# starkware-libs/stark-perpetual

Measured on AMD Instinct MI355X. Metric: pedersen_hashes_per_sec, higher is better.
Workload: dtype u32x9; 1 GPU; 2^16-leaf Pedersen Merkle rebuild per GPU (BASELINE.json configs[1]), 63 rebuilds in lockstep; tree_height=16, leaves_per_gpu=65536, calls_per_region=28, streams=2, window_bits=26, combine=none

## Files before the change

stark-perpetual_amd/csrc/pedersen.hip:

```cpp
#include <algorithm>
#include <cstdlib>
#include <cstring>
#include <map>
#include <vector>

#include "context.hpp"
#include "pedersen.hpp"
#include "quad.hpp"
#include "ragged_plan.hpp"

#ifndef SP_ACC_WAVES
#define SP_ACC_WAVES 1
#endif

namespace sp {

struct raw_aff {
  u256 x, y;
};
__device__ __forceinline__ raw_aff ld_raw(const aff_packed* e) {
  const uint4* q = reinterpret_cast<const uint4*>(e);
  const uint4 a = q[0], b = q[1], c = q[2], d = q[3];
  raw_aff r;
  r.x.w[0] = a.x; r.x.w[1] = a.y; r.x.w[2] = a.z; r.x.w[3] = a.w;
  r.x.w[4] = b.x; r.x.w[5] = b.y; r.x.w[6] = b.z; r.x.w[7] = b.w;
  r.y.w[0] = c.x; r.y.w[1] = c.y; r.y.w[2] = c.z; r.y.w[3] = c.w;
  r.y.w[4] = d.x; r.y.w[5] = d.y; r.y.w[6] = d.z; r.y.w[7] = d.w;
  return r;
}
__device__ __forceinline__ aff unpack_raw(const raw_aff& t) {
  aff r;
  r.x = fe_unpack(t.x);
  r.y = fe_unpack(t.y);
  return r;
}

struct bits512 {
  uint32_t w[16];
};
// ... 120 lines not shown
    acc = xyzz_mmadd<SP_SCAN_BULK>(unpack_raw(e0), q1);
    first = 2;
  } else {
    acc = xyzz_from_aff(unpack_raw(e0));
  }
  for (int i = first; i + 1 < nwin; ++i) {
    const aff q = signed_aff(n1, neg1);
    n1 = n2;
    neg1 = neg2;
    if (i + 2 < nwin) {
      const window_ref r = next_window(i + 2);
      n2 = ld_raw(r.entry);
      neg2 = r.negative;
    }
    acc = xyzz_madd<SP_SCAN_BULK>(acc, q);
  }
  if (nwin > 1) {
    fe X3, ZZ3;
    xyzz_madd_x_only<SP_SCAN_BULK>(acc, signed_aff(n1, neg1), X3, ZZ3);
    store_limbs(sX, plane, e, X3);
    store_limbs(sZZ, plane, e, ZZ3);
  } else {
    store_limbs(sX, plane, e, acc.X);
    store_limbs(sZZ, plane, e, acc.ZZ);
  }
  if (st != SP_HASH_OK) {
    if (status) status[e] = st;
    if (flag) atomicOr(flag, (unsigned)st);
  } else if (status) {
    status[e] = SP_HASH_OK;
  }
}

__global__ void __launch_bounds__(256, SP_ACC_WAVES)
ped_accumulate_kernel(const uint64_t* __restrict__ x, const uint64_t* __restrict__ y, size_t xstride,
                      size_t ystride, size_t n, const aff_packed* __restrict__ ped, int w0, int log2e,
                      int nwin, int32_t* __restrict__ sX, int32_t* __restrict__ sZZ,
                      uint8_t* __restrict__ status, unsigned* __restrict__ flag,
                      const int2* __restrict__ src, size_t plane) {
  bulk_accumulate(x, y, xstride, ystride, n, ped, w0, log2e, nwin, sX, sZZ, status, flag, src, plane,
                  (size_t)blockIdx.x * blockDim.x + threadIdx.x);
}

__device__ __forceinline__ fe shfl_xor_fe(const fe& v, int mask) {
  fe r;
#pragma unroll
  for (int i = 0; i < NL; ++i) r.l[i] = __shfl_xor(v.l[i], mask, 64);
  return r;
}
__device__ __forceinline__ uint32_t field_from_memory(const uint64_t* felt, int bit, int width) {
  const uint32_t* w = reinterpret_cast<const uint32_t*>(felt);
  const int wi = bit >> 5, sh = bit & 31;
  uint64_t two = (uint64_t)w[wi];
  if (wi + 1 < 8) two |= (uint64_t)w[wi + 1] << 32;
  return (uint32_t)(two >> sh) & ((1u << width) - 1u);
}
__device__ __forceinline__ uint32_t window_from_memory(const uint64_t* fx, const uint64_t* fy, int start,
                                                       int width) {
  if (start + width <= 252) return field_from_memory(fx, start, width);
  if (start >= 252) return field_from_memory(fy, start - 252, width);
  const int lo_n = 252 - start;
  return field_from_memory(fx, start, lo_n) | (field_from_memory(fy, 0, width - lo_n) << lo_n);
}

template <int LOG_L>
__device__ __forceinline__ xyzz split_accumulate(const uint64_t* fx, const uint64_t* fy, int sub,
                                                 const aff_packed* __restrict__ ped, int w0, int log2e,
                                                 int nwin) {
  constexpr int L = 1 << LOG_L;
  const int cnt_lo = nwin / L, extra = nwin % L;
  const int cnt = cnt_lo + (sub < extra ? 1 : 0);
  const int g0 = sub * cnt_lo + (sub < extra ? sub : extra);
  auto entry = [&](int g) {
    return window_entry(ped, g, window_from_memory(fx, fy, window_start(g, w0, log2e), window_width(g, w0, log2e)),
// ... 65 lines not shown
  u256 xa_plain;
  if (FUSED) {
    fe zz = acc.ZZ;
    if constexpr (LOG_L < 2) {
      if (fe_is_zero(zz)) {
        zz = FE_ONE_M;
        st = SP_HASH_UNHASHABLE;
      }
    }
    const fe zinv = fe_inv_shared_quad<(LOG_L >= 2 ? 0 : 2 - LOG_L), true>(zz, (int)(threadIdx.x & 3));
    if constexpr (LOG_L >= 2) {
      if (limbs_is_zero(zinv)) st = SP_HASH_UNHASHABLE;
    }
    xa_plain = fe_pack(fe_canon(fe_mul(acc.X, zinv)));
  }
  if (!active || sub != 0) return;
  if (!u256_lt(ld_u256(fx), U256_P) || !u256_lt(ld_u256(fy), U256_P)) st = SP_HASH_OUT_OF_RANGE;
  if (FUSED) {
    st_u256(out + 4 * e * ostride, xa_plain);
  } else {
    store_limbs(sX, plane, e, acc.X);
    store_limbs(sZZ, plane, e, acc.ZZ);
  }
  if (status) status[e] = st;
  if (st != SP_HASH_OK && flag) atomicOr(flag, (unsigned)st);
}

template <int LOG_L>
__global__ void __launch_bounds__(256, SP_ACC_WAVES)
ped_accumulate_mixed_kernel(const uint64_t* __restrict__ x, const uint64_t* __restrict__ y, size_t xstride,
                            size_t ystride, size_t n_bulk, size_t rem, unsigned bulk_blocks,
                            const aff_packed* __restrict__ ped, int w0, int log2e, int nwin,
                            int32_t* __restrict__ sX, int32_t* __restrict__ sZZ, uint8_t* __restrict__ status,
                            unsigned* __restrict__ flag, const int2* __restrict__ src, size_t plane) {
  if (blockIdx.x < bulk_blocks) {
    bulk_accumulate(x, y, xstride, ystride, n_bulk, ped, w0, log2e, nwin, sX, sZZ, status, flag, src, plane,
                    (size_t)blockIdx.x * blockDim.x + threadIdx.x);
    return;
  }
  constexpr int L = 1 << LOG_L;
  const size_t gt = (size_t)(blockIdx.x - bulk_blocks) * blockDim.x + threadIdx.x;
  const size_t e_raw = gt >> LOG_L;
  const int sub = (int)(gt & (L - 1));
  const bool active = e_raw < rem;
  const size_t e = n_bulk + (active ? e_raw : rem - 1);
  const uint64_t *fx, *fy;
  operand_pointers(x, y, xstride, ystride, src, e, fx, fy);
  const xyzz acc = split_accumulate<LOG_L>(fx, fy, sub, ped, w0, log2e, nwin);
  if (!active || sub != 0) return;
  uint8_t st = SP_HASH_OK;
  if (!u256_lt(ld_u256(fx), U256_P) || !u256_lt(ld_u256(fy), U256_P)) st = SP_HASH_OUT_OF_RANGE;
  store_limbs(sX, plane, e, acc.X);
  store_limbs(sZZ, plane, e, acc.ZZ);
  if (status) status[e] = st;
  if (st != SP_HASH_OK && flag) atomicOr(flag, (unsigned)st);
}

template <int LOG_Q, bool SPARSE>
__device__ __forceinline__ u256 quad_hash(const uint64_t* fx, const uint64_t* fy, int mode, const aff_packed* __restrict__ cpts,
                                          int cx, int cy, const aff_packed* __restrict__ ped, int w0, int log2e,
                                          int nwin_plan, int g, bool* unhashable) {
  constexpr int QUADS = 1 << LOG_Q;
  const int q = g >> 2, k = g & 3;
  int nwin = nwin_plan, first_real = 0;
  if constexpr (SPARSE) {
    nwin = mode == 0 ? nwin_plan : 1 + nwin_plan - (mode == 1 ? cx : cy);
    first_real = mode == 1 ? cx - 1 : (mode == 2 ? -1 : 0);
  }
  auto entry = [&](int v) {
    if constexpr (SPARSE) {
      if (mode != 0 && v == 0) return unpack_raw(ld_raw(cpts + (mode - 1)));
    }
    const int w = first_real + v;
    const window_ref r =
// ... 230 lines not shown
        if (st != SP_HASH_OK && flag) atomicOr(flag, (unsigned)st);
      }
    }
    __syncthreads();
    h = slot[grp];
  }
}

__global__ void __launch_bounds__(256)
ped_fold_ragged_scatter_kernel(const uint64_t* __restrict__ work, const uint64_t* __restrict__ lone, bool sided,
                               const uint32_t* __restrict__ off, const uint32_t* __restrict__ perm,
                               const uint32_t* __restrict__ step_off, const uint8_t* __restrict__ step_status, size_t n,
                               unsigned* __restrict__ flag, uint8_t* __restrict__ status, uint64_t* __restrict__ out,
                               const uint64_t* __restrict__ expect, size_t estride, uint8_t* __restrict__ verdict) {
  const size_t k = (size_t)blockIdx.x * blockDim.x + threadIdx.x;
  if (k >= n) return;
  const uint32_t c = perm[k];
  const uint32_t o0 = off[c], steps = off[c + 1] - o0 - (sided ? 0 : 1);
  uint8_t st = SP_HASH_OK;
  u256 v;
  if (steps == 0) {
    v = ld_u256(lone + 4 * (size_t)(sided ? c : o0));
    if (!u256_lt(v, U256_P)) st = SP_HASH_OUT_OF_RANGE;
    if (st != SP_HASH_OK && flag) atomicOr(flag, (unsigned)st);
  } else {
    v = ld_u256(work + 4 * k);
    for (uint32_t s = 0; s < steps; ++s) st |= step_status[(size_t)step_off[s] + k];
  }
  fold_result<true>(c, v, st, out, status, expect, estride, verdict);
}

__global__ void __launch_bounds__(256)
ped_top_kernel(uint64_t* __restrict__ cur, size_t n_in, int n_levels, const aff_packed* __restrict__ ped, int w0, int log2e,
               int nwin_plan, unsigned* __restrict__ flag) {
  constexpr int LANES = 32, GROUPS = 256 / LANES;
  __shared__ uint64_t slot[2][GROUPS][4];
  const int g = (int)(threadIdx.x % LANES), grp = (int)(threadIdx.x / LANES);
  const size_t b = blockIdx.x;
  const int chunk = 1 << n_levels;
  uint64_t* out = cur + 4 * n_in;
  size_t n_out = n_in >> 1;
  int share = 4 - n_levels;
  for (int t = 0; t < n_levels; ++t, ++share) {
    const int cnt = chunk >> (t + 1);
    const int i = grp >> share;
    const bool writer = g == 0 && (grp & ((1 << share) - 1)) == 0;
    const uint64_t *fx, *fy;
    if (t == 0) {
      fx = cur + 4 * ((size_t)chunk * b + 2 * (size_t)i);
      fy = fx + 4;
    } else {
      fx = slot[(t - 1) & 1][2 * i];
      fy = slot[(t - 1) & 1][2 * i + 1];
    }
    bool unhashable;
    const u256 xa = quad_hash<3, false>(fx, fy, 0, nullptr, 0, 0, ped, w0, log2e, nwin_plan, g, &unhashable);
    uint8_t st = unhashable ? SP_HASH_UNHASHABLE : SP_HASH_OK;
    if (t == 0 && writer && (!u256_lt(ld_u256(fx), U256_P) || !u256_lt(ld_u256(fy), U256_P))) st = SP_HASH_OUT_OF_RANGE;
    if (writer) {
      uint32_t* sl = reinterpret_cast<uint32_t*>(slot[t & 1][i]);
#pragma unroll
      for (int w = 0; w < 8; ++w) sl[w] = xa.w[w];
      st_u256(out + 4 * ((size_t)cnt * b + (size_t)i), xa);
      if (st != SP_HASH_OK && flag) atomicOr(flag, (unsigned)st);
    }
    __syncthreads();
    out += 4 * n_out;
    n_out >>= 1;
  }
}

__global__ void __launch_bounds__(256)
ped_finish_kernel(const int32_t* __restrict__ sX, int32_t* __restrict__ sZZ, int32_t* __restrict__ sPre,
                  size_t n, size_t T, uint64_t* __restrict__ out, size_t ostride,
                  uint8_t* __restrict__ status, unsigned* __restrict__ flag) {
  const size_t t = (size_t)blockIdx.x * blockDim.x + threadIdx.x;
  if (t >= T) return;
  const size_t cnt = t < n ? (n - t + T - 1) / T : 0;
  fe run = FE_ONE_M;
  if (cnt > 0) {
    fe znext = load_limbs(sZZ, n, t);
#pragma unroll 1
    for (size_t j = 0; j < cnt; ++j) {
      const size_t e = t + j * T;
      const fe z = znext;
      if (j + 1 < cnt) znext = load_limbs(sZZ, n, e + T);
      store_limbs(sPre, n, e, run);
      run = fe_mul(run, z);
    }
  }
  if (fe_is_zero(run)) {
    run = FE_ONE_M;
#pragma unroll 1
    for (size_t e = t; e < n; e += T) {
      fe z = load_limbs(sZZ, n, e);
      if (fe_is_zero(z)) {
        z = FE_ONE_M;
        store_limbs(sZZ, n, e, z);
        if (status) status[e] = SP_HASH_UNHASHABLE;
        if (flag) atomicOr(flag, (unsigned)SP_HASH_UNHASHABLE);
      }
      store_limbs(sPre, n, e, run);
      run = fe_mul(run, z);
    }
  }
  size_t e = cnt > 0 ? t + (cnt - 1) * T : 0;
  fe zn = run, pn = run, xn = run;
  if (cnt > 0) {
    zn = load_limbs(sZZ, n, e);
    pn = load_limbs(sPre, n, e);
    xn = load_limbs(sX, n, e);
  }
  fe inv = fe_inv_shared_quad<2, true>(run, (int)(threadIdx.x & 3));
#pragma unroll 1
  for (size_t j = cnt; j-- > 0;) {
    const fe z = zn, pre = pn, xv = xn;
    const size_t cur = t + j * T;
    if (j > 0) {
      zn = load_limbs(sZZ, n, cur - T);
      pn = load_limbs(sPre, n, cur - T);
      xn = load_limbs(sX, n, cur - T);
    }
    const fe zinv = fe_mul(inv, pre);
    inv = fe_mul(inv, z);
    const fe xa = fe_mul(xv, zinv);
    st_u256(out + 4 * cur * ostride, fe_pack(fe_canon(xa)));
  }
}

template <bool Z_IN_LDS>
__global__ void __launch_bounds__(256)
ped_finish_lds_kernel(const int32_t* __restrict__ sX, int32_t* __restrict__ sZZ, size_t n, size_t T,
                      uint64_t* __restrict__ out, size_t ostride, uint8_t* __restrict__ status,
                      unsigned* __restrict__ flag, int kmax) {
  extern __shared__ int32_t fin_lds[];
  int32_t* lpre = fin_lds;
  int32_t* lz = fin_lds + (size_t)kmax * NL * 256;
  auto lds_put = [&](int32_t* base, size_t j, const fe& v) {
#pragma unroll
    for (int k = 0; k < NL; ++k) base[((j * NL + k) << 8) + threadIdx.x] = v.l[k];
  };
  auto lds_get = [&](const int32_t* base, size_t j) {
    fe v;
#pragma unroll
    for (int k = 0; k < NL; ++k) v.l[k] = base[((j * NL + k) << 8) + threadIdx.x];
    return v;
  };
  const size_t t = (size_t)blockIdx.x * blockDim.x + threadIdx.x;
  if (t >= T) return;
  const size_t cnt = t < n ? (n - t + T - 1) / T : 0;
  fe run = FE_ONE_M;
  if (cnt > 0) {
    fe znext = load_limbs(sZZ, n, t);
#pragma unroll 1
    for (size_t j = 0; j < cnt; ++j) {
      const fe z = znext;
      if (j + 1 < cnt) znext = load_limbs(sZZ, n, t + (j + 1) * T);
      lds_put(lpre, j, run);
      if (Z_IN_LDS) lds_put(lz, j, z);
      run = fe_mul(run, z);
    }
  }
  if (fe_is_zero(run)) {
    run = FE_ONE_M;
    size_t j = 0;
#pragma unroll 1
    for (size_t e = t; e < n; e += T, ++j) {
      fe z = load_limbs(sZZ, n, e);
      if (fe_is_zero(z)) {
        z = FE_ONE_M;
        store_limbs(sZZ, n, e, z);
        if (status) status[e] = SP_HASH_UNHASHABLE;
        if (flag) atomicOr(flag, (unsigned)SP_HASH_UNHASHABLE);
      }
      lds_put(lpre, j, run);
      if (Z_IN_LDS) lds_put(lz, j, z);
      run = fe_mul(run, z);
    }
  }
  size_t e = cnt > 0 ? t + (cnt - 1) * T : 0;
  fe zn = run, xn = run;
  if (cnt > 0) {
    if (!Z_IN_LDS) zn = load_limbs(sZZ, n, e);
    xn = load_limbs(sX, n, e);
  }
  fe inv = fe_inv_shared_quad<2, true>(run, (int)(threadIdx.x & 3));
#pragma unroll 1
  for (size_t j = cnt; j-- > 0;) {
    const fe z = Z_IN_LDS ? lds_get(lz, j) : zn, xv = xn;
    const fe pre = lds_get(lpre, j);
    const size_t cur = t + j * T;
    if (j > 0) {
      if (!Z_IN_LDS) zn = load_limbs(sZZ, n, cur - T);
      xn = load_limbs(sX, n, cur - T);
    }
    const fe zinv = fe_mul(inv, pre);
    inv = fe_mul(inv, z);
    const fe xa = fe_mul(xv, zinv);
    st_u256(out + 4 * cur * ostride, fe_pack(fe_canon(xa)));
  }
}

__global__ void __launch_bounds__(128)
ped_point_kernel(const uint64_t* __restrict__ x, const uint64_t* __restrict__ y, size_t n,
                 const aff_packed* __restrict__ ped, int w0, int log2e, int nwin,
                 uint64_t* __restrict__ ox, uint64_t* __restrict__ oy, uint8_t* __restrict__ status) {
  size_t e = (size_t)blockIdx.x * blockDim.x + threadIdx.x;
  if (e >= n) e = n - 1;
  u256 sx = ld_u256(x + 4 * e);
  u256 sy = ld_u256(y + 4 * e);
  if (!u256_lt(sx, U256_P) || !u256_lt(sy, U256_P)) {
    status[e] = SP_HASH_OUT_OF_RANGE;
    return;
  }
  bits512 str = concat_xy(sx, sy);
  xyzz acc = xyzz_from_aff(ld_aff(ped + pop_bits(str, w0)));
  for (int g = 1; g < nwin; ++g) {
    const window_ref r = window_entry(ped, g, pop_bits(str, log2e + 1), w0, log2e);
    acc = xyzz_madd(acc, signed_aff(ld_raw(r.entry), r.negative));
  }
  if (fe_is_zero(acc.ZZ)) {
    status[e] = SP_HASH_UNHASHABLE;
    return;
  }
  const fe izzz = fe_inv(acc.ZZZ);
  st_u256(ox + 4 * e, fe_pack(fe_from_mont(fe_mul(acc.X, fe_sqr(fe_mul(acc.ZZ, izzz))))));
  st_u256(oy + 4 * e, fe_pack(fe_from_mont(fe_mul(acc.Y, izzz))));
// ... 107 lines not shown

static size_t g_finish_lanes = getenv("STARKPERP_FINISH_LANES") ? (size_t)atoll(getenv("STARKPERP_FINISH_LANES")) : 65536;
static size_t parse_split_lanes() {
  const char* e = getenv("STARKPERP_SPLIT_LANES");
  long long v = e ? atoll(e) : 65536;
  if (v < 256) v = 256;
  if (v > (1ll << 24)) v = 1ll << 24;
  return ((size_t)v + 255) & ~(size_t)255;
}
static size_t g_split_lanes = parse_split_lanes();
static bool g_finish_lds = getenv("STARKPERP_NO_FINISH_LDS") == nullptr;
static int finish_lds_ready() {
  static std::map<int, int> done;
  int dev = -1;
  if (hipGetDevice(&dev) != hipSuccess) return SP_ERR_HIP;
  auto it = done.find(dev);
  if (it != done.end()) return it->second;
  const int want = 16 * NL * 256 * (int)sizeof(int32_t);
  hipError_t e = hipFuncSetAttribute(reinterpret_cast<const void*>(ped_finish_lds_kernel<true>),
                                     hipFuncAttributeMaxDynamicSharedMemorySize, want);
  if (e == hipSuccess)
    e = hipFuncSetAttribute(reinterpret_cast<const void*>(ped_finish_lds_kernel<false>),
                            hipFuncAttributeMaxDynamicSharedMemorySize, want);
  if (e != hipSuccess) (void)hipGetLastError();
  return done[dev] = (e == hipSuccess ? SP_OK : SP_ERR_HIP);
}
static size_t finish_threads(size_t n) {
  size_t K = (n + g_finish_lanes - 1) / g_finish_lanes;
  if (K < 1) K = 1;
  if (K > 32) K = 32;
  return ((n + K - 1) / K + 3) & ~(size_t)3;
}

void release_ragged_stage();
void release_pedersen_state() {
  for (auto& kv : g_stream_scratch) kv.second.release();
  g_stream_scratch.clear();
  release_ragged_stage();
  for (hipEvent_t e : g_prof.ev) (void)hipEventDestroy(e);
  g_prof.ev.clear();
  g_prof.units.clear();
  g_prof.used = 0;
  g_prof.enabled = false;
}

void constant_window_counts(const PedPlan& p, int& cx, int& cy) {
  cx = cy = 0;
  for (int g = 0; g < p.nwin; ++g) {
    if (p.start[g] + p.bits[g] <= 252) ++cx;
    if (p.start[g] >= 252) ++cy;
  }
}
static bool sparse_class(const PedPlan& plan, int log_q, int& cx, int& cy) {
  if (!g_sparse_enabled || (log_q != 1 && log_q != 2)) return false;
  constant_window_counts(plan, cx, cy);
  const int shortest = 1 + plan.nwin - (cx > cy ? cx : cy);
  return cx >= 1 && cy >= 1 && shortest >= (2 << log_q);
}
int enqueue_partial_points(const uint64_t* felts, int count, aff_packed* out, hipStream_t st, bool* usable) {
  Context& c = ctx();
  int cx, cy;
  constant_window_counts(c.plan, cx, cy);
  *usable = cx >= 1 && cy >= 1 && count > 0;
  if (!*usable) return SP_OK;
  hipLaunchKernelGGL(ped_partial_kernel, dim3((unsigned)((2 * count + 63) / 64)), dim3(64), 0, st, felts, count, c.ped,
                     (int)c.plan.bits[0], c.plan.log2e, c.plan.nwin, cx, cy, out);
  SP_HIP(hipGetLastError());
  return SP_OK;
}

static int enqueue_pedersen_impl(const uint64_t* x, size_t xs, const uint64_t* y, size_t ys, uint64_t* out,
                                 size_t os, uint8_t* status, unsigned* flag, size_t n, hipStream_t st,
                                 const Scratch& s, const int2* src, const aff_packed* cpts);
int enqueue_pedersen(const uint64_t* x, size_t xs, const uint64_t* y, size_t ys, uint64_t* out,
                     size_t os, uint8_t* status, unsigned* flag, size_t n, hipStream_t st,
                     const Scratch& s, const int2* src) {
  return enqueue_pedersen_impl(x, xs, y, ys, out, os, status, flag, n, st, s, src, nullptr);
}
int enqueue_pedersen_sparse(const uint64_t* x, const uint64_t* y, uint64_t* out, unsigned* flag, size_t n,
                            hipStream_t st, const Scratch& s, const int2* src, const aff_packed* cpts) {
  return enqueue_pedersen_impl(x, 1, y, 1, out, 1, nullptr, flag, n, st, s, src, cpts);
}
static bool g_path_fusion = getenv("STARKPERP_NO_PATH_FUSION") == nullptr;
static bool g_top_fusion = getenv("STARKPERP_NO_TOP_FUSION") == nullptr;
static bool g_chain_fusion = getenv("STARKPERP_NO_CHAIN_FUSION") == nullptr;
int enqueue_pedersen_chain(const uint64_t* first, const uint64_t* words, long long word_stride, size_t n, size_t steps,
                           bool h_right, uint64_t* out, unsigned* flag, hipStream_t st, bool* done) {
  *done = false;
  Context& c = ctx();
  const int w0 = c.plan.bits[0], log2e = c.plan.log2e, nwin = c.plan.nwin;
  if (!g_chain_fusion || n == 0 || steps < 2 || steps > 0x7fffffffull) return SP_OK;
  const QuadShape q = quad_shape(n, nwin);
  if (q.log_q == 0) return SP_OK;
  dispatch_quad(q.log_q, false, [&](auto Q, auto) {
    hipLaunchKernelGGL((ped_chain_kernel<decltype(Q)::value>), dim3(q.blocks), dim3(256), 0, st, first, words, word_stride,
                       n, (int)steps, h_right, c.ped, w0, log2e, nwin, flag, out, q.dup);
  });
  SP_HIP(hipGetLastError());
  *done = true;
  return SP_OK;
}
int enqueue_pedersen_top(uint64_t* cur, size_t n_in, unsigned remaining, unsigned* flag, hipStream_t st, int* levels_done) {
  *levels_done = 0;
  Context& c = ctx();
  const int nwin = c.plan.nwin;
  if (!g_top_fusion || !g_quad_enabled || nwin > 64 || nwin < 16 || remaining < 2 || n_in / 2 > g_quad_max || n_in < 4) return SP_OK;
  const int L = remaining < 4 ? (int)remaining : 4;
  const unsigned blocks = (unsigned)(n_in >> L);
  hipLaunchKernelGGL(ped_top_kernel, dim3(blocks), dim3(256), 0, st, cur, n_in, L, c.ped, (int)c.plan.bits[0], c.plan.log2e,
                     nwin, flag);
  SP_HIP(hipGetLastError());
  *levels_done = L;
  return SP_OK;
}
int enqueue_pedersen_path(uint64_t* felts, const uint64_t* emp, unsigned* flag, size_t n, hipStream_t st,
                          const int2* src_all, const PathLevels& pl, const aff_packed* cpts_tree, bool* done) {
  *done = false;
  Context& c = ctx();
  const int w0 = c.plan.bits[0], log2e = c.plan.log2e, nwin = c.plan.nwin;
  if (!g_path_fusion || n == 0 || pl.n_levels < 2) return SP_OK;
  const QuadShape q = quad_shape(n, nwin);
  if (q.log_q == 0) return SP_OK;
  int cx = 0, cy = 0;
  const bool sparse = cpts_tree != nullptr && sparse_class(c.plan, q.log_q, cx, cy);
  dispatch_quad(q.log_q, sparse, [&](auto Q, auto S) {
    hipLaunchKernelGGL((ped_path_kernel<decltype(Q)::value, decltype(S)::value>), dim3(q.blocks), dim3(256), 0, st, felts,
                       emp, n, c.ped, w0, log2e, nwin, flag, src_all, pl, q.dup, sparse ? cpts_tree : nullptr, cx, cy);
  });
  SP_HIP(hipGetLastError());
  *done = true;
  return SP_OK;
}

static int enqueue_pedersen_impl(const uint64_t* x, size_t xs, const uint64_t* y, size_t ys, uint64_t* out,
                                 size_t os, uint8_t* status, unsigned* flag, size_t n, hipStream_t st,
                                 const Scratch& s, const int2* src, const aff_packed* cpts) {
  if (n == 0) return SP_OK;
  Context& c = ctx();
  bool prof = false;
  const int w0 = c.plan.bits[0], log2e = c.plan.log2e, nwin = c.plan.nwin;
  int log_l = 0;
  bool fused = false;
  if (g_split_enabled) {
    if (n * 8 <= g_split_lanes) log_l = 3;
    else if (n * 4 <= g_split_lanes) log_l = 2;
    else if (n * 2 <= g_split_lanes) log_l = 1;
    while (log_l > 0 && nwin < (2 << log_l)) --log_l;
  }
  const QuadShape q = quad_shape(n, nwin);
  if (q.log_q != 0) {
    int cx = 0, cy = 0;
    const bool sparse = cpts != nullptr && src != nullptr && sparse_class(c.plan, q.log_q, cx, cy);
    dispatch_quad(q.log_q, sparse, [&](auto Q, auto S) {
      hipLaunchKernelGGL((ped_quad_kernel<decltype(Q)::value, decltype(S)::value>), dim3(q.blocks), dim3(256), 0, st, x, y,
                         xs, ys, n, c.ped, w0, log2e, nwin, status, flag, src, out, os, q.dup, cpts, cx, cy);
    });
    fused = true;
  } else if (log_l == 0 && !(g_split_enabled && g_fuse_enabled && n <= 65536)) {
    size_t n_bulk = n, rem = 0;
    int rem_l = 0;
    if (g_level_split && g_split_enabled && n > g_split_lanes && (n % g_split_lanes) != 0 &&
        (n % g_split_lanes) * 2 <= g_split_lanes) {
      rem = n % g_split_lanes;
      rem_l = rem * 8 <= g_split_lanes ? 3 : (rem * 4 <= g_split_lanes ? 2 : 1);
      while (rem_l > 0 && nwin < (2 << rem_l)) --rem_l;
      if (rem_l == 0) rem = 0;
      n_bulk = n - rem;
    }
    if (rem == 0) {
      prof = g_prof.enabled && g_prof.used + 2 <= g_prof.ev.size() && n > 65536;
      if (prof) (void)hipEventRecord(g_prof.ev[g_prof.used], st);
      hipLaunchKernelGGL(ped_accumulate_kernel, dim3((unsigned)((n_bulk + 255) / 256)), dim3(256), 0, st, x, y, xs, ys,
                         n_bulk, c.ped, w0, log2e, nwin, s.X, s.ZZ, status, flag, src, n);
    } else {
      const unsigned bulk_blocks = (unsigned)(n_bulk / 256);
      const unsigned rblocks = (unsigned)(((rem << rem_l) + 255) / 256);
#define SP_LAUNCH_MIXED(LOGL)                                                                                     \
  hipLaunchKernelGGL((ped_accumulate_mixed_kernel<LOGL>), dim3(bulk_blocks + rblocks), dim3(256), 0, st, x, y, xs, \
                     ys, n_bulk, rem, bulk_blocks, c.ped, w0, log2e, nwin, s.X, s.ZZ, status, flag, src, n)
      if (rem_l == 3) SP_LAUNCH_MIXED(3);
      else if (rem_l == 2) SP_LAUNCH_MIXED(2);
      else SP_LAUNCH_MIXED(1);
#undef SP_LAUNCH_MIXED
    }
    if (prof) {
      (void)hipEventRecord(g_prof.ev[g_prof.used + 1], st);
      g_prof.units.push_back(n);
      g_prof.used += 2;
    }
  } else {
    const unsigned blocks = (unsigned)(((n << log_l) + 255) / 256);
    fused = g_fuse_enabled && (n << log_l) <= 65536;
#define SP_LAUNCH_SPLIT(LOGL, FUSEDV)                                                                      \
  hipLaunchKernelGGL((ped_accumulate_split_kernel<LOGL, FUSEDV>), dim3(blocks), dim3(256), 0, st, x, y, xs, \
                     ys, n, c.ped, w0, log2e, nwin, s.X, s.ZZ, status, flag, src, out, os, n)
    if (log_l == 0) SP_LAUNCH_SPLIT(0, true);
    else if (log_l == 3) { if (fused) SP_LAUNCH_SPLIT(3, true); else SP_LAUNCH_SPLIT(3, false); }
    else if (log_l == 2) { if (fused) SP_LAUNCH_SPLIT(2, true); else SP_LAUNCH_SPLIT(2, false); }
    else { if (fused) SP_LAUNCH_SPLIT(1, true); else SP_LAUNCH_SPLIT(1, false); }
#undef SP_LAUNCH_SPLIT
  }
  if (!fused) {
    const size_t T = finish_threads(n);
    const unsigned tpb = T >= 256 ? 256 : 64;
    const unsigned blocksB = (unsigned)((T + tpb - 1) / tpb);
    const size_t kmax = (n + T - 1) / T;
    if (g_finish_lds && tpb == 256 && kmax >= 2 && kmax <= 16 && finish_lds_ready() == SP_OK) {
      const bool z_too = kmax <= 8;
      const size_t lds_bytes = kmax * NL * 256 * sizeof(int32_t) * (z_too ? 2 : 1);
      if (z_too) hipLaunchKernelGGL((ped_finish_lds_kernel<true>), dim3(blocksB), dim3(256), lds_bytes, st, s.X, s.ZZ, n, T,
                                    out, os, status, flag, (int)kmax);
      else hipLaunchKernelGGL((ped_finish_lds_kernel<false>), dim3(blocksB), dim3(256), lds_bytes, st, s.X, s.ZZ, n, T,
                              out, os, status, flag, (int)kmax);
    } else {
      hipLaunchKernelGGL(ped_finish_kernel, dim3(blocksB), dim3(tpb), 0, st, s.X, s.ZZ, s.Pre, n, T, out,
                         os, status, flag);
    }
  }
  SP_HIP(hipGetLastError());
  return SP_OK;
}

static bool g_chain_ragged = getenv("STARKPERP_NO_CHAIN_RAGGED") == nullptr;
static bool g_path_fold = getenv("STARKPERP_NO_PATH_FOLD") == nullptr;
struct RaggedStage {
  PinnedBuffer host;
  hipEvent_t copied = nullptr;
  bool pending = false;
};
static std::map<StreamKey, RaggedStage> g_ragged_stage;
void release_ragged_stage() {
  for (auto& kv : g_ragged_stage) {
    if (kv.second.copied) (void)hipEventDestroy(kv.second.copied);
    kv.second.host.release();
  }
  g_ragged_stage.clear();
}
int stage_copy(std::initializer_list<Piece> pieces, void* dev, hipStream_t st) {
  RaggedStage& rs = g_ragged_stage[stream_key(st)];
  if (rs.pending) {
    SP_HIP(hipEventSynchronize(rs.copied));
    rs.pending = false;
  }
  if (rs.copied == nullptr) SP_HIP(hipEventCreateWithFlags(&rs.copied, hipEventDisableTiming));
  size_t bytes = 0;
  for (const Piece& p : pieces) bytes += p.bytes;
  SP_HIP(rs.host.reserve(bytes));
  size_t at = 0;
  for (const Piece& p : pieces) {
    if (p.bytes) std::memcpy((char*)rs.host.ptr + at, p.ptr, p.bytes);
    at += p.bytes;
// ... 400 lines not shown
  SP_HIP(c.io.reserve((n_elems + 2) * 32 + 64));
  uint64_t* d_el = (uint64_t*)c.io.ptr;
  uint64_t* d_a = d_el + 4 * n_elems;
  uint64_t* d_b = d_a + 4;
  SP_HIP(hipMemcpy(d_el, elems, n_elems * 32, hipMemcpyHostToDevice));
  Scratch s;
  int rc = get_scratch(1, s, 0);
  if (rc != SP_OK) return rc;
  SP_HIP(hipMemsetAsync(s.flag, 0, sizeof(unsigned), 0));
  const uint64_t* h = d_el + 4 * (n_elems - 1);
  uint64_t* nxt = d_a;
  bool fused = false;
  if (n_elems >= 3) {
    rc = enqueue_pedersen_chain(h, d_el + 4 * (n_elems - 2), -1, 1, n_elems - 1, true, d_a, s.flag, 0, &fused);
    if (rc != SP_OK) return rc;
    if (fused) h = d_a;
  }
  for (size_t i = n_elems - 1; !fused && i-- > 0;) {
    rc = enqueue_pedersen(d_el + 4 * i, 1, h, 1, nxt, 1, nullptr, s.flag, 1, 0, s, nullptr);
    if (rc != SP_OK) return rc;
    h = nxt;
    nxt = (nxt == d_a) ? d_b : d_a;
  }
  SP_HIP(hipDeviceSynchronize());
  SP_HIP(hipMemcpy(out, h, 32, hipMemcpyDeviceToHost));
  if (status) {
    unsigned f = 0;
    SP_HIP(hipMemcpy(&f, s.flag, sizeof(unsigned), hipMemcpyDeviceToHost));
    *status = (uint8_t)f;
  }
  return SP_OK;
}

int sp_merkle_forest_dev(uint64_t* levels, size_t n_trees, unsigned height, uint8_t* status,
                         void* stream) {
  CtxByPointer sp_ctx_sel__(levels);
  SP_REQUIRE_READY();
  if (n_trees == 0) return SP_OK;
  if (height > 40 || (n_trees >> (40 - height)) != 0) { set_error("forest too large"); return SP_ERR_BAD_ARGUMENT; }
  Context& c = ctx();
  ctx_lock lk(c.mu);
  hipStream_t st = (hipStream_t)stream;
  const size_t n0 = n_trees << height;
  Scratch s;
  int rc = get_scratch(n0 / 2 + 1, s, st);
  if (rc != SP_OK) return rc;
  SP_HIP(hipMemsetAsync(s.flag, 0, sizeof(unsigned), st));
  uint64_t* cur = levels;
  size_t n = n0;
  for (unsigned k = 0; k < height;) {
    int fused = 0;
    rc = enqueue_pedersen_top(cur, n, height - k, s.flag, st, &fused);
    if (rc != SP_OK) return rc;
    if (fused > 0) {
      for (int j = 0; j < fused; ++j, n >>= 1) cur += 4 * n;
      k += (unsigned)fused;
      continue;
    }
    uint64_t* nxt = cur + 4 * n;
    rc = enqueue_pedersen(cur, 2, cur + 4, 2, nxt, 1, nullptr, s.flag, n / 2, st, s, nullptr);
    if (rc != SP_OK) return rc;
    cur = nxt;
    ++k;
    n >>= 1;
  }
  if (status) SP_HIP(hipMemcpyAsync(status, s.flag, 1, hipMemcpyDeviceToHost, st));
  return SP_OK;
}

int sp_merkle_build_dev(uint64_t* levels, unsigned height, uint8_t* status, void* stream) {
  return sp_merkle_forest_dev(levels, 1, height, status, stream);
}

int sp_commit_rows_dev(const uint64_t* cols, size_t n_rows, size_t n_cols, uint64_t* levels, uint8_t* status,
                       void* stream) {
  CtxByPointer sp_ctx_sel__(cols);
  SP_REQUIRE_READY();
  if (n_rows == 0 || (n_rows & (n_rows - 1)) != 0 || n_cols == 0) {
    set_error("rows must be a power of two, columns at least one");
    return SP_ERR_BAD_ARGUMENT;
  }
  ctx_lock lk(ctx().mu);
  unsigned height = 0;
  while (((size_t)1 << height) < n_rows) ++height;
  uint8_t st_chain = 0, st_tree = 0;
  int rc = sp_pedersen_chains_dev(cols, n_rows, n_cols, levels, status ? &st_chain : nullptr, stream);
  if (rc != SP_OK) return rc;
  rc = sp_merkle_build_dev(levels, height, status ? &st_tree : nullptr, stream);
  if (rc != SP_OK) return rc;
  if (status) {
    SP_HIP(hipStreamSynchronize((hipStream_t)stream));
    *status = st_chain | st_tree;
  }
  return SP_OK;
}

int sp_merkle_root(const uint64_t* leaves, unsigned height, uint64_t* root, uint64_t* levels_out,
                   uint8_t* status) {
  SP_REQUIRE_READY();
// ... 20 lines not shown
```

Before: 1.024 billion hashes/s.

## Pipeline forest level finishes into next accumulate launches and double-buffer status flags

Adds an optional forest pipeline that splits each of the lower Merkle levels into two parts and runs one part's batched-inverse finish as extra blocks inside the next part's accumulate kernel. This hides the separate finish-kernel launch and its tail under accumulate work. The per-call flag memset is also replaced by a pair of flag words that alternate between calls, with the top kernel clearing the next word, which removes one memset launch per rebuild. The pipeline is off unless STARKPERP_FINISH_PIPELINE is set, but the flag double-buffering runs by default. It also adds extra scratch planes and more complex indexing.

Result: no change. 1.023 billion hashes/s (-0.1%).

```diff
diff --git a/stark-perpetual_amd/csrc/forest_pipeline.hpp b/stark-perpetual_amd/csrc/forest_pipeline.hpp
--- /dev/null
+++ b/stark-perpetual_amd/csrc/forest_pipeline.hpp
@@ -0,0 +1,27 @@
+#pragma once
+#include <cstddef>
+
+namespace sp {
+
+struct ForestPipeline {
+  unsigned levels = 0;
+  size_t n_last = 0;
+  size_t b_last = 0;
+  size_t hashes(unsigned k) const { return n_last << (levels - 1 - k); }
+  size_t part_b(unsigned k) const { return b_last << (levels - 1 - k); }
+  size_t part_a(unsigned k) const { return hashes(k) - part_b(k); }
+};
+
+inline ForestPipeline forest_pipeline(size_t n_trees, unsigned height, size_t round) {
+  ForestPipeline p;
+  if (n_trees == 0 || height == 0 || round == 0) return p;
+  unsigned big = 0;
+  while (big < height && (n_trees << (height - 1 - big)) / round >= 4) ++big;
+  if (big == 0) return p;
+  p.levels = big < height ? big + 1 : big;
+  p.n_last = n_trees << (height - p.levels);
+  p.b_last = p.n_last / round / 2 * round;
+  return p;
+}
+
+}
diff --git a/stark-perpetual_amd/csrc/pedersen.hip b/stark-perpetual_amd/csrc/pedersen.hip
--- a/stark-perpetual_amd/csrc/pedersen.hip
+++ b/stark-perpetual_amd/csrc/pedersen.hip
@@ -5,6 +5,7 @@
 #include <vector>
 
 #include "context.hpp"
+#include "forest_pipeline.hpp"
 #include "pedersen.hpp"
 #include "quad.hpp"
 #include "ragged_plan.hpp"
@@ -191,14 +192,88 @@
   }
 }
 
+struct FinishPart {
+  const int32_t* sX;
+  int32_t* sZZ;
+  int32_t* sPre;
+  size_t plane, n, T;
+  uint64_t* out;
+  size_t ostride;
+  uint8_t* status;
+  unsigned blocks;
+};
+__device__ __forceinline__ void finish_part(const FinishPart& f, size_t t, unsigned* __restrict__ flag) {
+  const int32_t* __restrict__ sX = f.sX;
+  int32_t* __restrict__ sZZ = f.sZZ;
+  int32_t* __restrict__ sPre = f.sPre;
+  uint64_t* __restrict__ out = f.out;
+  uint8_t* __restrict__ status = f.status;
+  const size_t plane = f.plane, n = f.n, T = f.T, ostride = f.ostride;
+  if (t >= T) return;
+  const size_t cnt = t < n ? (n - t + T - 1) / T : 0;
+  fe run = FE_ONE_M;
+  if (cnt > 0) {
+    fe znext = load_limbs(sZZ, plane, t);
+#pragma unroll 1
+    for (size_t j = 0; j < cnt; ++j) {
+      const size_t e = t + j * T;
+      const fe z = znext;
+      if (j + 1 < cnt) znext = load_limbs(sZZ, plane, e + T);
+      store_limbs(sPre, plane, e, run);
+      run = fe_mul(run, z);
+    }
+  }
+  if (fe_is_zero(run)) {
+    run = FE_ONE_M;
+#pragma unroll 1
+    for (size_t e = t; e < n; e += T) {
+      fe z = load_limbs(sZZ, plane, e);
+      if (fe_is_zero(z)) {
+        z = FE_ONE_M;
+        store_limbs(sZZ, plane, e, z);
+        if (status) status[e] = SP_HASH_UNHASHABLE;
+        if (flag) atomicOr(flag, (unsigned)SP_HASH_UNHASHABLE);
+      }
+      store_limbs(sPre, plane, e, run);
+      run = fe_mul(run, z);
+    }
+  }
+  size_t e = cnt > 0 ? t + (cnt - 1) * T : 0;
+  fe zn = run, pn = run, xn = run;
+  if (cnt > 0) {
+    zn = load_limbs(sZZ, plane, e);
+    pn = load_limbs(sPre, plane, e);
+    xn = load_limbs(sX, plane, e);
+  }
+  fe inv = fe_inv_shared_quad<2, true>(run, (int)(threadIdx.x & 3));
+#pragma unroll 1
+  for (size_t j = cnt; j-- > 0;) {
+    const fe z = zn, pre = pn, xv = xn;
+    const size_t cur = t + j * T;
+    if (j > 0) {
+      zn = load_limbs(sZZ, plane, cur - T);
+      pn = load_limbs(sPre, plane, cur - T);
+      xn = load_limbs(sX, plane, cur - T);
+    }
+    const fe zinv = fe_mul(inv, pre);
+    inv = fe_mul(inv, z);
+    const fe xa = fe_mul(xv, zinv);
+    st_u256(out + 4 * cur * ostride, fe_pack(fe_canon(xa)));
+  }
+}
+
 __global__ void __launch_bounds__(256, SP_ACC_WAVES)
 ped_accumulate_kernel(const uint64_t* __restrict__ x, const uint64_t* __restrict__ y, size_t xstride,
                       size_t ystride, size_t n, const aff_packed* __restrict__ ped, int w0, int log2e,
                       int nwin, int32_t* __restrict__ sX, int32_t* __restrict__ sZZ,
                       uint8_t* __restrict__ status, unsigned* __restrict__ flag,
-                      const int2* __restrict__ src, size_t plane) {
+                      const int2* __restrict__ src, size_t plane, FinishPart fin) {
+  if (blockIdx.x < fin.blocks) {
+    finish_part(fin, (size_t)blockIdx.x * blockDim.x + threadIdx.x, flag);
+    return;
+  }
   bulk_accumulate(x, y, xstride, ystride, n, ped, w0, log2e, nwin, sX, sZZ, status, flag, src, plane,
-                  (size_t)blockIdx.x * blockDim.x + threadIdx.x);
+                  (size_t)(blockIdx.x - fin.blocks) * blockDim.x + threadIdx.x);
 }
 
 __device__ __forceinline__ fe shfl_xor_fe(const fe& v, int mask) {
@@ -330,14 +405,19 @@
                             size_t ystride, size_t n_bulk, size_t rem, unsigned bulk_blocks,
                             const aff_packed* __restrict__ ped, int w0, int log2e, int nwin,
                             int32_t* __restrict__ sX, int32_t* __restrict__ sZZ, uint8_t* __restrict__ status,
-                            unsigned* __restrict__ flag, const int2* __restrict__ src, size_t plane) {
-  if (blockIdx.x < bulk_blocks) {
+                            unsigned* __restrict__ flag, const int2* __restrict__ src, size_t plane, FinishPart fin) {
+  if (blockIdx.x < fin.blocks) {
+    finish_part(fin, (size_t)blockIdx.x * blockDim.x + threadIdx.x, flag);
+    return;
+  }
+  const unsigned bid = blockIdx.x - fin.blocks;
+  if (bid < bulk_blocks) {
     bulk_accumulate(x, y, xstride, ystride, n_bulk, ped, w0, log2e, nwin, sX, sZZ, status, flag, src, plane,
-                    (size_t)blockIdx.x * blockDim.x + threadIdx.x);
+                    (size_t)bid * blockDim.x + threadIdx.x);
     return;
   }
   constexpr int L = 1 << LOG_L;
-  const size_t gt = (size_t)(blockIdx.x - bulk_blocks) * blockDim.x + threadIdx.x;
+  const size_t gt = (size_t)(bid - bulk_blocks) * blockDim.x + threadIdx.x;
   const size_t e_raw = gt >> LOG_L;
   const int sub = (int)(gt & (L - 1));
   const bool active = e_raw < rem;
@@ -634,9 +714,10 @@
 
 __global__ void __launch_bounds__(256)
 ped_top_kernel(uint64_t* __restrict__ cur, size_t n_in, int n_levels, const aff_packed* __restrict__ ped, int w0, int log2e,
-               int nwin_plan, unsigned* __restrict__ flag) {
+               int nwin_plan, unsigned* __restrict__ flag, unsigned* __restrict__ clear) {
   constexpr int LANES = 32, GROUPS = 256 / LANES;
   __shared__ uint64_t slot[2][GROUPS][4];
+  if (clear != nullptr && blockIdx.x == 0 && threadIdx.x == 0) *clear = 0;
   const int g = (int)(threadIdx.x % LANES), grp = (int)(threadIdx.x / LANES);
   const size_t b = blockIdx.x;
   const int chunk = 1 << n_levels;
@@ -673,66 +754,16 @@
 }
 
 __global__ void __launch_bounds__(256)
-ped_finish_kernel(const int32_t* __restrict__ sX, int32_t* __restrict__ sZZ, int32_t* __restrict__ sPre,
-                  size_t n, size_t T, uint64_t* __restrict__ out, size_t ostride,
-                  uint8_t* __restrict__ status, unsigned* __restrict__ flag) {
-  const size_t t = (size_t)blockIdx.x * blockDim.x + threadIdx.x;
-  if (t >= T) return;
-  const size_t cnt = t < n ? (n - t + T - 1) / T : 0;
-  fe run = FE_ONE_M;
-  if (cnt > 0) {
-    fe znext = load_limbs(sZZ, n, t);
-#pragma unroll 1
-    for (size_t j = 0; j < cnt; ++j) {
-      const size_t e = t + j * T;
-      const fe z = znext;
-      if (j + 1 < cnt) znext = load_limbs(sZZ, n, e + T);
-      store_limbs(sPre, n, e, run);
-      run = fe_mul(run, z);
-    }
-  }
-  if (fe_is_zero(run)) {
-    run = FE_ONE_M;
-#pragma unroll 1
-    for (size_t e = t; e < n; e += T) {
-      fe z = load_limbs(sZZ, n, e);
-      if (fe_is_zero(z)) {
-        z = FE_ONE_M;
-        store_limbs(sZZ, n, e, z);
-        if (status) status[e] = SP_HASH_UNHASHABLE;
-        if (flag) atomicOr(flag, (unsigned)SP_HASH_UNHASHABLE);
-      }
-      store_limbs(sPre, n, e, run);
-      run = fe_mul(run, z);
-    }
-  }
-  size_t e = cnt > 0 ? t + (cnt - 1) * T : 0;
-  fe zn = run, pn = run, xn = run;
-  if (cnt > 0) {
-    zn = load_limbs(sZZ, n, e);
-    pn = load_limbs(sPre, n, e);
-    xn = load_limbs(sX, n, e);
-  }
-  fe inv = fe_inv_shared_quad<2, true>(run, (int)(threadIdx.x & 3));
-#pragma unroll 1
-  for (size_t j = cnt; j-- > 0;) {
-    const fe z = zn, pre = pn, xv = xn;
-    const size_t cur = t + j * T;
-    if (j > 0) {
-      zn = load_limbs(sZZ, n, cur - T);
-      pn = load_limbs(sPre, n, cur - T);
-      xn = load_limbs(sX, n, cur - T);
-    }
-    const fe zinv = fe_mul(inv, pre);
-    inv = fe_mul(inv, z);
-    const fe xa = fe_mul(xv, zinv);
-    st_u256(out + 4 * cur * ostride, fe_pack(fe_canon(xa)));
-  }
+ped_finish_kernel(const int32_t* __restrict__ sX, int32_t* __restrict__ sZZ, int32_t* __restrict__ sPre, size_t plane,
+                  size_t n, size_t T, uint64_t* __restrict__ out, size_t ostride, uint8_t* __restrict__ status,
+                  unsigned* __restrict__ flag) {
+  const FinishPart f{sX, sZZ, sPre, plane, n, T, out, ostride, status, 0};
+  finish_part(f, (size_t)blockIdx.x * blockDim.x + threadIdx.x, flag);
 }
 
 template <bool Z_IN_LDS>
 __global__ void __launch_bounds__(256)
-ped_finish_lds_kernel(const int32_t* __restrict__ sX, int32_t* __restrict__ sZZ, size_t n, size_t T,
+ped_finish_lds_kernel(const int32_t* __restrict__ sX, int32_t* __restrict__ sZZ, size_t plane, size_t n, size_t T,
                       uint64_t* __restrict__ out, size_t ostride, uint8_t* __restrict__ status,
                       unsigned* __restrict__ flag, int kmax) {
   extern __shared__ int32_t fin_lds[];
@@ -753,11 +784,11 @@
   const size_t cnt = t < n ? (n - t + T - 1) / T : 0;
   fe run = FE_ONE_M;
   if (cnt > 0) {
-    fe znext = load_limbs(sZZ, n, t);
+    fe znext = load_limbs(sZZ, plane, t);
 #pragma unroll 1
     for (size_t j = 0; j < cnt; ++j) {
       const fe z = znext;
-      if (j + 1 < cnt) znext = load_limbs(sZZ, n, t + (j + 1) * T);
+      if (j + 1 < cnt) znext = load_limbs(sZZ, plane, t + (j + 1) * T);
       lds_put(lpre, j, run);
       if (Z_IN_LDS) lds_put(lz, j, z);
       run = fe_mul(run, z);
@@ -768,10 +799,10 @@
     size_t j = 0;
 #pragma unroll 1
     for (size_t e = t; e < n; e += T, ++j) {
-      fe z = load_limbs(sZZ, n, e);
+      fe z = load_limbs(sZZ, plane, e);
       if (fe_is_zero(z)) {
         z = FE_ONE_M;
-        store_limbs(sZZ, n, e, z);
+        store_limbs(sZZ, plane, e, z);
         if (status) status[e] = SP_HASH_UNHASHABLE;
         if (flag) atomicOr(flag, (unsigned)SP_HASH_UNHASHABLE);
       }
@@ -783,8 +814,8 @@
   size_t e = cnt > 0 ? t + (cnt - 1) * T : 0;
   fe zn = run, xn = run;
   if (cnt > 0) {
-    if (!Z_IN_LDS) zn = load_limbs(sZZ, n, e);
-    xn = load_limbs(sX, n, e);
+    if (!Z_IN_LDS) zn = load_limbs(sZZ, plane, e);
+    xn = load_limbs(sX, plane, e);
   }
   fe inv = fe_inv_shared_quad<2, true>(run, (int)(threadIdx.x & 3));
 #pragma unroll 1
@@ -793,8 +824,8 @@
     const fe pre = lds_get(lpre, j);
     const size_t cur = t + j * T;
     if (j > 0) {
-      if (!Z_IN_LDS) zn = load_limbs(sZZ, n, cur - T);
-      xn = load_limbs(sX, n, cur - T);
+      if (!Z_IN_LDS) zn = load_limbs(sZZ, plane, cur - T);
+      xn = load_limbs(sX, plane, cur - T);
     }
     const fe zinv = fe_mul(inv, pre);
     inv = fe_mul(inv, z);
@@ -968,10 +999,18 @@
   return ((n + K - 1) / K + 3) & ~(size_t)3;
 }
 
+struct ForestFlags {
+  DeviceBuffer words;
+  unsigned turn = 0;
+  bool dirty = true;
+};
+static std::map<StreamKey, ForestFlags> g_forest_flags;
 void release_ragged_stage();
 void release_pedersen_state() {
   for (auto& kv : g_stream_scratch) kv.second.release();
   g_stream_scratch.clear();
+  for (auto& kv : g_forest_flags) kv.second.words.release();
+  g_forest_flags.clear();
   release_ragged_stage();
   for (hipEvent_t e : g_prof.ev) (void)hipEventDestroy(e);
   g_prof.ev.clear();
@@ -1036,7 +1075,8 @@
   *done = true;
   return SP_OK;
 }
-int enqueue_pedersen_top(uint64_t* cur, size_t n_in, unsigned remaining, unsigned* flag, hipStream_t st, int* levels_done) {
+static int enqueue_pedersen_top(uint64_t* cur, size_t n_in, unsigned remaining, unsigned* flag, unsigned* clear, hipStream_t st,
+                                int* levels_done) {
   *levels_done = 0;
   Context& c = ctx();
   const int nwin = c.plan.nwin;
@@ -1044,7 +1084,7 @@
   const int L = remaining < 4 ? (int)remaining : 4;
   const unsigned blocks = (unsigned)(n_in >> L);
   hipLaunchKernelGGL(ped_top_kernel, dim3(blocks), dim3(256), 0, st, cur, n_in, L, c.ped, (int)c.plan.bits[0], c.plan.log2e,
-                     nwin, flag);
+                     nwin, flag, (unsigned)L == remaining ? clear : nullptr);
   SP_HIP(hipGetLastError());
   *levels_done = L;
   return SP_OK;
@@ -1068,12 +1108,66 @@
   return SP_OK;
 }
 
+static void launch_accumulate(const uint64_t* x, size_t xs, const uint64_t* y, size_t ys, uint8_t* status, unsigned* flag,
+                              size_t n, hipStream_t st, int32_t* sX, int32_t* sZZ, size_t plane, const int2* src,
+                              const FinishPart& fin) {
+  Context& c = ctx();
+  const int w0 = c.plan.bits[0], log2e = c.plan.log2e, nwin = c.plan.nwin;
+  size_t n_bulk = n, rem = 0;
+  int rem_l = 0;
+  if (g_level_split && g_split_enabled && n > g_split_lanes && (n % g_split_lanes) != 0 &&
+      (n % g_split_lanes) * 2 <= g_split_lanes) {
+    rem = n % g_split_lanes;
+    rem_l = rem * 8 <= g_split_lanes ? 3 : (rem * 4 <= g_split_lanes ? 2 : 1);
+    while (rem_l > 0 && nwin < (2 << rem_l)) --rem_l;
+    if (rem_l == 0) rem = 0;
+    n_bulk = n - rem;
+  }
+  if (rem == 0) {
+    const bool prof = g_prof.enabled && g_prof.used + 2 <= g_prof.ev.size() && n > 65536;
+    if (prof) (void)hipEventRecord(g_prof.ev[g_prof.used], st);
+    hipLaunchKernelGGL(ped_accumulate_kernel, dim3(fin.blocks + (unsigned)((n_bulk + 255) / 256)), dim3(256), 0, st, x, y,
+                       xs, ys, n_bulk, c.ped, w0, log2e, nwin, sX, sZZ, status, flag, src, plane, fin);
+    if (prof) {
+      (void)hipEventRecord(g_prof.ev[g_prof.used + 1], st);
+      g_prof.units.push_back(n);
+      g_prof.used += 2;
+    }
+  } else {
+    const unsigned bulk_blocks = (unsigned)(n_bulk / 256);
+    const unsigned rblocks = (unsigned)(((rem << rem_l) + 255) / 256);
+#define SP_LAUNCH_MIXED(LOGL)                                                                                          \
+  hipLaunchKernelGGL((ped_accumulate_mixed_kernel<LOGL>), dim3(fin.blocks + bulk_blocks + rblocks), dim3(256), 0, st, x, \
+                     y, xs, ys, n_bulk, rem, bulk_blocks, c.ped, w0, log2e, nwin, sX, sZZ, status, flag, src, plane, fin)
+    if (rem_l == 3) SP_LAUNCH_MIXED(3);
+    else if (rem_l == 2) SP_LAUNCH_MIXED(2);
+    else SP_LAUNCH_MIXED(1);
+#undef SP_LAUNCH_MIXED
+  }
+}
+static void launch_finish(const int32_t* sX, int32_t* sZZ, int32_t* sPre, size_t plane, size_t n, uint64_t* out, size_t os,
+                          uint8_t* status, unsigned* flag, hipStream_t st) {
+  const size_t T = finish_threads(n);
+  const unsigned tpb = T >= 256 ? 256 : 64;
+  const unsigned blocksB = (unsigned)((T + tpb - 1) / tpb);
+  const size_t kmax = (n + T - 1) / T;
+  if (g_finish_lds && tpb == 256 && kmax >= 2 && kmax <= 16 && finish_lds_ready() == SP_OK) {
+    const bool z_too = kmax <= 8;
+    const size_t lds_bytes = kmax * NL * 256 * sizeof(int32_t) * (z_too ? 2 : 1);
+    if (z_too) hipLaunchKernelGGL((ped_finish_lds_kernel<true>), dim3(blocksB), dim3(256), lds_bytes, st, sX, sZZ, plane, n, T,
+                                  out, os, status, flag, (int)kmax);
+    else hipLaunchKernelGGL((ped_finish_lds_kernel<false>), dim3(blocksB), dim3(256), lds_bytes, st, sX, sZZ, plane, n, T,
+                            out, os, status, flag, (int)kmax);
+  } else {
+    hipLaunchKernelGGL(ped_finish_kernel, dim3(blocksB), dim3(tpb), 0, st, sX, sZZ, sPre, plane, n, T, out, os, status, flag);
+  }
+}
+
 static int enqueue_pedersen_impl(const uint64_t* x, size_t xs, const uint64_t* y, size_t ys, uint64_t* out,
                                  size_t os, uint8_t* status, unsigned* flag, size_t n, hipStream_t st,
                                  const Scratch& s, const int2* src, const aff_packed* cpts) {
   if (n == 0) return SP_OK;
   Context& c = ctx();
-  bool prof = false;
   const int w0 = c.plan.bits[0], log2e = c.plan.log2e, nwin = c.plan.nwin;
   int log_l = 0;
   bool fused = false;
@@ -1093,37 +1187,7 @@
     });
     fused = true;
   } else if (log_l == 0 && !(g_split_enabled && g_fuse_enabled && n <= 65536)) {
-    size_t n_bulk = n, rem = 0;
-    int rem_l = 0;
-    if (g_level_split && g_split_enabled && n > g_split_lanes && (n % g_split_lanes) != 0 &&
-        (n % g_split_lanes) * 2 <= g_split_lanes) {
-      rem = n % g_split_lanes;
-      rem_l = rem * 8 <= g_split_lanes ? 3 : (rem * 4 <= g_split_lanes ? 2 : 1);
-      while (rem_l > 0 && nwin < (2 << rem_l)) --rem_l;
-      if (rem_l == 0) rem = 0;
-      n_bulk = n - rem;
-    }
-    if (rem == 0) {
-      prof = g_prof.enabled && g_prof.used + 2 <= g_prof.ev.size() && n > 65536;
-      if (prof) (void)hipEventRecord(g_prof.ev[g_prof.used], st);
-      hipLaunchKernelGGL(ped_accumulate_kernel, dim3((unsigned)((n_bulk + 255) / 256)), dim3(256), 0, st, x, y, xs, ys,
-                         n_bulk, c.ped, w0, log2e, nwin, s.X, s.ZZ, status, flag, src, n);
-    } else {
-      const unsigned bulk_blocks = (unsigned)(n_bulk / 256);
-      const unsigned rblocks = (unsigned)(((rem << rem_l) + 255) / 256);
-#define SP_LAUNCH_MIXED(LOGL)                                                                                     \
-  hipLaunchKernelGGL((ped_accumulate_mixed_kernel<LOGL>), dim3(bulk_blocks + rblocks), dim3(256), 0, st, x, y, xs, \
-                     ys, n_bulk, rem, bulk_blocks, c.ped, w0, log2e, nwin, s.X, s.ZZ, status, flag, src, n)
-      if (rem_l == 3) SP_LAUNCH_MIXED(3);
-      else if (rem_l == 2) SP_LAUNCH_MIXED(2);
-      else SP_LAUNCH_MIXED(1);
-#undef SP_LAUNCH_MIXED
-    }
-    if (prof) {
-      (void)hipEventRecord(g_prof.ev[g_prof.used + 1], st);
-      g_prof.units.push_back(n);
-      g_prof.used += 2;
-    }
+    launch_accumulate(x, xs, y, ys, status, flag, n, st, s.X, s.ZZ, n, src, FinishPart{});
   } else {
     const unsigned blocks = (unsigned)(((n << log_l) + 255) / 256);
     fused = g_fuse_enabled && (n << log_l) <= 65536;
@@ -1136,23 +1200,7 @@
     else { if (fused) SP_LAUNCH_SPLIT(1, true); else SP_LAUNCH_SPLIT(1, false); }
 #undef SP_LAUNCH_SPLIT
   }
-  if (!fused) {
-    const size_t T = finish_threads(n);
-    const unsigned tpb = T >= 256 ? 256 : 64;
-    const unsigned blocksB = (unsigned)((T + tpb - 1) / tpb);
-    const size_t kmax = (n + T - 1) / T;
-    if (g_finish_lds && tpb == 256 && kmax >= 2 && kmax <= 16 && finish_lds_ready() == SP_OK) {
-      const bool z_too = kmax <= 8;
-      const size_t lds_bytes = kmax * NL * 256 * sizeof(int32_t) * (z_too ? 2 : 1);
-      if (z_too) hipLaunchKernelGGL((ped_finish_lds_kernel<true>), dim3(blocksB), dim3(256), lds_bytes, st, s.X, s.ZZ, n, T,
-                                    out, os, status, flag, (int)kmax);
-      else hipLaunchKernelGGL((ped_finish_lds_kernel<false>), dim3(blocksB), dim3(256), lds_bytes, st, s.X, s.ZZ, n, T,
-                              out, os, status, flag, (int)kmax);
-    } else {
-      hipLaunchKernelGGL(ped_finish_kernel, dim3(blocksB), dim3(tpb), 0, st, s.X, s.ZZ, s.Pre, n, T, out,
-                         os, status, flag);
-    }
-  }
+  if (!fused) launch_finish(s.X, s.ZZ, s.Pre, n, n, out, os, status, flag, st);
   SP_HIP(hipGetLastError());
   return SP_OK;
 }
@@ -1619,6 +1667,48 @@
   return SP_OK;
 }
 
+static bool g_finish_pipeline = getenv("STARKPERP_FINISH_PIPELINE") != nullptr && getenv("STARKPERP_NO_FINISH_PIPELINE") == nullptr;
+static size_t g_pipeline_k = getenv("STARKPERP_PIPELINE_K") ? (size_t)atoll(getenv("STARKPERP_PIPELINE_K")) : 32;
+static size_t plane_bytes(size_t n) { return ((9 * n * sizeof(int32_t)) + 255) & ~(size_t)255; }
+static int enqueue_forest_pipeline(uint64_t* levels, const ForestPipeline& pp, const Scratch& s, char* odd, hipStream_t st) {
+  const unsigned L = pp.levels - 1;
+  int32_t* const X1 = (int32_t*)odd;
+  int32_t* const ZZ1 = (int32_t*)(odd + plane_bytes(pp.hashes(1)));
+  struct Part {
+    const uint64_t* in;
+    uint64_t* out;
+    int32_t *X, *ZZ, *Pre;
+    size_t plane, n;
+  };
+  auto part = [&](unsigned k, bool back) {
+    uint64_t* in = levels;
+    for (unsigned j = 0; j < k; ++j) in += 8 * pp.hashes(j);
+    const size_t base = back ? pp.part_a(k) : 0, nk = pp.hashes(k);
+    return Part{in + 8 * base, in + 8 * nk + 4 * base, ((k & 1) ? X1 : s.X) + base, ((k & 1) ? ZZ1 : s.ZZ) + base,
+                s.Pre + base, nk, back ? pp.part_b(k) : pp.part_a(k)};
+  };
+  auto finish_role = [&](const Part& p) {
+    size_t T = finish_threads(p.n);
+    if (g_pipeline_k >= 1) {
+      const size_t K = g_pipeline_k > 32 ? 32 : g_pipeline_k;
+      T = ((p.n + K - 1) / K + 3) & ~(size_t)3;
+    }
+    return FinishPart{p.X, p.ZZ, p.Pre, p.plane, p.n, T, p.out, 1, nullptr, (unsigned)((T + 255) / 256)};
+  };
+  auto accumulate = [&](const Part& p, const FinishPart& fin) {
+    launch_accumulate(p.in, 2, p.in + 4, 2, nullptr, s.flag, p.n, st, p.X, p.ZZ, p.plane, nullptr, fin);
+  };
+  accumulate(part(0, false), FinishPart{});
+  for (unsigned k = 0; k <= L; ++k) {
+    accumulate(part(k, true), finish_role(part(k, false)));
+    if (k < L) accumulate(part(k + 1, false), finish_role(part(k, true)));
+  }
+  const Part last = part(L, true);
+  launch_finish(last.X, last.ZZ, last.Pre, last.plane, last.n, last.out, 1, nullptr, s.flag, st);
+  SP_HIP(hipGetLastError());
+  return SP_OK;
+}
+
 int sp_merkle_forest_dev(uint64_t* levels, size_t n_trees, unsigned height, uint8_t* status,
                          void* stream) {
   CtxByPointer sp_ctx_sel__(levels);
@@ -1629,19 +1719,40 @@
   ctx_lock lk(c.mu);
   hipStream_t st = (hipStream_t)stream;
   const size_t n0 = n_trees << height;
+  const ForestPipeline pp = g_finish_pipeline ? forest_pipeline(n_trees, height, g_split_lanes) : ForestPipeline{};
   Scratch s;
-  int rc = get_scratch(n0 / 2 + 1, s, st);
+  char* odd = nullptr;
+  int rc = pp.levels >= 2 ? get_scratch_tail(n0 / 2 + 1, 2 * plane_bytes(pp.hashes(1)), s, &odd, st) : get_scratch(n0 / 2 + 1, s, st);
   if (rc != SP_OK) return rc;
-  SP_HIP(hipMemsetAsync(s.flag, 0, sizeof(unsigned), st));
+  ForestFlags& ff = g_forest_flags[stream_key(st)];
+  hipStreamCaptureStatus capturing = hipStreamCaptureStatusNone;
+  (void)hipStreamIsCapturing(st, &capturing);
+  if (ff.words.ptr == nullptr) SP_HIP(ff.words.reserve(2 * sizeof(unsigned)));
+  unsigned* const words = (unsigned*)ff.words.ptr;
+  if (ff.dirty || capturing != hipStreamCaptureStatusNone) {
+    SP_HIP(hipMemsetAsync(words, 0, 2 * sizeof(unsigned), st));
+    ff.turn = 0;
+  }
+  ff.dirty = true;
+  s.flag = words + ff.turn;
+  unsigned* const next_flag = words + (ff.turn ^ 1);
+  bool cleared = false;
   uint64_t* cur = levels;
   size_t n = n0;
-  for (unsigned k = 0; k < height;) {
+  unsigned k = 0;
+  if (pp.levels >= 2) {
+    rc = enqueue_forest_pipeline(levels, pp, s, odd, st);
+    if (rc != SP_OK) return rc;
+    for (; k < pp.levels; ++k, n >>= 1) cur += 4 * n;
+  }
+  while (k < height) {
     int fused = 0;
-    rc = enqueue_pedersen_top(cur, n, height - k, s.flag, st, &fused);
+    rc = enqueue_pedersen_top(cur, n, height - k, s.flag, next_flag, st, &fused);
     if (rc != SP_OK) return rc;
     if (fused > 0) {
       for (int j = 0; j < fused; ++j, n >>= 1) cur += 4 * n;
       k += (unsigned)fused;
+      cleared = k == height;
       continue;
     }
     uint64_t* nxt = cur + 4 * n;
@@ -1651,7 +1762,10 @@
     ++k;
     n >>= 1;
   }
+  if (!cleared) SP_HIP(hipMemsetAsync(next_flag, 0, sizeof(unsigned), st));
   if (status) SP_HIP(hipMemcpyAsync(status, s.flag, 1, hipMemcpyDeviceToHost, st));
+  ff.turn ^= 1;
+  ff.dirty = capturing != hipStreamCaptureStatusNone;
   return SP_OK;
 }
 
```
